# TritonDataCenter/registrar

Hardware: NVIDIA H100
Metric: service-records/sec (higher is better)
Workload: dtype u8

## Files before the change

registrar_b200/csrc/regk_api.cu:

```cuda
#include <cuda_runtime.h>

#include <algorithm>
#include <cstdarg>
#include <cstdio>
#include <cstdlib>
#include <cstring>
#include <map>
#include <mutex>
#include <string>
#include <vector>

#include "../../include/regk.h"
#include "regk_kernels.cuh"
#include "regk_gather.cuh"
#include "regk_peersync.cuh"
#include "regk_service.cuh"
#include "regk_jute.cuh"
#include "regk_decode.cuh"
#include "regk_parents.cuh"
#include "regk_types.hpp"

using namespace regk;

namespace {

thread_local std::string g_create_error;

struct DevBuf {
    void *p = nullptr;
    size_t cap = 0;
};

struct HostBuf {
    void *p = nullptr;
    size_t cap = 0;
};

}

struct regk_ctx {
    int device = 0;
    cudaStream_t own_stream = nullptr;
    cudaStream_t stream = nullptr;
    std::string err;
    int sm_count = 0;
    int max_smem_optin = 0;

    std::vector<std::string> types;
    std::vector<uint8_t> blob_host;
    DevBuf blob_dev;
    uint32_t max_type_q = 0;

    DevBuf in[11];
    DevBuf path_bytes, path_off, json_bytes, json_off, off32_p, off32_j;
    HostBuf h_path_bytes, h_path_off, h_json_bytes, h_json_off, h_running;
    cudaStream_t s_h2d = nullptr, s_d2h = nullptr;
    struct HostSet {
        DevBuf in[11];
        DevBuf path_bytes, path_off, json_bytes, json_off, off32_p, off32_j;
        HostBuf h_path_bytes, h_path_off, h_json_bytes, h_json_off;
        cudaEvent_t e_in = nullptr, e_out = nullptr;
    };
    HostSet hset[2];
    uint64_t hseq = 0;
    uint32_t *h_gather_flag = nullptr;
    double json_mean_seen = 0.0;
    uint64_t json_est_seen = 0;
    bool json_learning = true;
    regk_job job{};
    bool job_bound = false;
    unsigned long long job_seq = 0;
    DevBuf job_bases;
    unsigned long long *h_job_bases = nullptr;
    const uint8_t *last_path_bytes = nullptr;
    const unsigned long long *last_path_off = nullptr;
    uint64_t last_n = 0;
    const uint8_t *last_json_bytes = nullptr;
    const unsigned long long *last_json_off = nullptr;
    uint64_t last_json_n = 0;
// ... 280 lines not shown
            jp.base_out = hp.running + c + 1;
        }
        if (do_path) {
            pp.n = cn;
            pp.rec0 = r0;
            pp.domain_off += r0;
            if (pp.host_off) {
                pp.host_off += r0;
                pp.off_bias = alias ? r0 : 2 * r0;
            } else if (!alias) {
                pp.host_bytes += r0 * (size_t)stride;
                pp.host_limit -= r0 * (uint64_t)stride;
                pp.off_bias = r0 * (uint64_t)(stride + 2);
            } else {
                pp.off_bias = r0;
            }
            pp.out_off += r0;
            pp.tile_total += t0;
            pp.super_total += c * hp.nsuper_chunk;
            const JsonParams side = do_json ? jp : JsonParams{};
            if (alias)
                regk_path_kernel<true, false><<<(unsigned)ct, TILE, path_smem, s>>>(pp, side);
            else
                regk_path_kernel<false, false><<<(unsigned)ct, TILE, path_smem, s>>>(pp, side);
            CK(cudaGetLastError());
            launches++;
        }
        if (do_json) {
            if (!do_path) {
                regk_json_len_kernel<<<(unsigned)std::min<uint64_t>(ct, (uint64_t)ctx->sm_count * 8), TILE, 0, s>>>(jp, (uint32_t)ct);
                CK(cudaGetLastError());
                launches++;
            }
            regk_json_kernel<<<(unsigned)ct, TILE, json_smem, s>>>(jp);
            CK(cudaGetLastError());
            launches++;
            CK(cudaMemcpyAsync(h_running + c + 1, hp.running + c + 1, 8, cudaMemcpyDeviceToHost, s));
        }
        if (c + 1 == hp.nchunks)
            CK(cudaMemcpyAsync(h_status, d_status, sizeof(DevStatus), cudaMemcpyDeviceToHost, s));
        CK(cudaEventRecord(e_done, s));
    }
    h_running[0] = 0;
    for (uint64_t c = 0; c < hp.nchunks; c++) {
        const uint64_t r0 = c * hp.chunk, r1 = std::min(n, r0 + hp.chunk);
        cudaError_t e = cudaEventSynchronize(ctx->pipe_events[3 * c + 1]);
        if (e != cudaSuccess)
            return fail(ctx, REGK_ERR_CUDA, "kernel execution failed: %s", cudaGetErrorString(e));
        const bool last = c + 1 == hp.nchunks;
        if (do_path) {
            const uint64_t lo = path_cf(r0), hi = std::min<uint64_t>(path_cf(r1), hp.path_cap);
            if (hi > lo)
                CK(cudaMemcpyAsync((uint8_t *)ctx->h_path_bytes.p + lo, (uint8_t *)ctx->path_bytes.p + lo, hi - lo,
                    cudaMemcpyDeviceToHost, ctx->s_d2h));
            CK(cudaMemcpyAsync((uint64_t *)ctx->h_path_off.p + r0, (uint64_t *)ctx->path_off.p + r0, (r1 - r0 + (last ? 1 : 0)) * 8,
                cudaMemcpyDeviceToHost, ctx->s_d2h));
        }
        if (do_json) {
            const uint64_t lo = h_running[c], hi = std::min<uint64_t>(h_running[c + 1], hp.json_cap);
            if (hi > lo)
                CK(cudaMemcpyAsync((uint8_t *)ctx->h_json_bytes.p + lo, (uint8_t *)ctx->json_bytes.p + lo, hi - lo,
                    cudaMemcpyDeviceToHost, ctx->s_d2h));
            CK(cudaMemcpyAsync((uint64_t *)ctx->h_json_off.p + r0, (uint64_t *)ctx->json_off.p + r0, (r1 - r0 + (last ? 1 : 0)) * 8,
                cudaMemcpyDeviceToHost, ctx->s_d2h));
        }
    }
    cudaError_t e = cudaStreamSynchronize(ctx->s_d2h);
// ... 226 lines not shown
        cudaStreamDestroy(ctx->own_stream);
    delete ctx;
}

int regk_set_stream(regk_ctx *ctx, void *cuda_stream)
{
    if (!ctx)
        return REGK_ERR_INVALID_ARG;
    if (ctx->pending)
        return fail(ctx, REGK_ERR_STATE, "regk_set_stream: a batch is still pending; call regk_finish first");
    ctx->stream = cuda_stream ? (cudaStream_t)cuda_stream : ctx->own_stream;
    return REGK_OK;
}

int regk_set_option(regk_ctx *ctx, const char *name, int64_t value)
{
    if (!ctx || !name)
        return REGK_ERR_INVALID_ARG;
    static const char *known[] = {"async", "force_generic", "dom_cap", "json_out_cap", "chunk_records", "time_every", "offsets32", nullptr};
    for (const char **k = known; *k; k++)
        if (!strcmp(*k, name)) {
            ctx->opt[name] = value;
            return REGK_OK;
        }
    return fail(ctx, REGK_ERR_INVALID_ARG, "regk_set_option: unknown option '%s'", name);
}

int64_t regk_get_option(const regk_ctx *ctx, const char *name)
{
    if (!ctx || !name)
        return -1;
    if (!strcmp(name, "sm_count"))
        return ctx->sm_count;
    return opt_get(ctx, name, 0);
}

int regk_set_types(regk_ctx *ctx, const char *const *types, const uint32_t *lens, uint32_t ntypes)
{
    if (!ctx || (!types && ntypes))
        return fail(ctx, REGK_ERR_INVALID_ARG, "regk_set_types: NULL argument");
    if (ntypes > 255)
        return fail(ctx, REGK_ERR_INVALID_ARG, "regk_set_types: at most 255 types (type_id is one byte)");
    if (ctx->pending)
        return fail(ctx, REGK_ERR_STATE, "regk_set_types: a batch is still pending");
    CK(cudaSetDevice(ctx->device));
    std::vector<std::string> raw(ntypes);
    for (uint32_t i = 0; i < ntypes; i++)
        raw[i].assign(types[i], lens ? lens[i] : strlen(types[i]));
    std::vector<uint8_t> blob;
    uint32_t maxq = 0;
    std::string why;
    const int brc = build_type_blob(raw, &blob, &maxq, &why);
    if (brc)
        return fail(ctx, brc == 1 ? REGK_ERR_OUT_OF_DOMAIN : REGK_ERR_INVALID_ARG, "regk_set_types: %s", why.c_str());
    int rc = ensure_dev(ctx, ctx->blob_dev, blob.size());
    if (rc)
        return rc;
    CK(cudaMemcpyAsync(ctx->blob_dev.p, blob.data(), blob.size(), cudaMemcpyHostToDevice, ctx->stream));
    CK(cudaStreamSynchronize(ctx->stream));
    ctx->types = raw;
    ctx->blob_host = blob;
    ctx->max_type_q = maxq;
    ctx->json_mean_seen = 0.0;
    ctx->json_learning = true;
    return REGK_OK;
}
// ... 420 lines not shown
        pp.tile_total = (uint32_t *)(wk + totals_p_off);
        pp.super_total = (unsigned long long *)(wk + super_p_off);
        pp.status = d_status;
        pp.dom_limit = dom_len;
        pp.host_limit = host_len;
        pp.force_generic = force_generic;
        const uint64_t mean_dom_tile = std::min<uint64_t>(dom_len, dom_len * TILE / std::max<uint64_t>(n, 1)) + 1;
        uint32_t dom_cap = (uint32_t)opt_get(ctx, "dom_cap", 0);
        if (!dom_cap)
            dom_cap = (uint32_t)std::min<uint64_t>(std::max<uint64_t>(align16(mean_dom_tile * 5 / 4 + 384), 2048), 49152);
        dom_cap = (uint32_t)((dom_cap + 127) & ~127u);
        uint32_t host_cap = 0;
        if (!alias) {
            const uint64_t mean_host_tile = pp.host_off ? std::min<uint64_t>(host_len, host_len * TILE / std::max<uint64_t>(n, 1)) + 1
                                                        : (uint64_t)TILE * b->host_stride;
            host_cap = (uint32_t)std::min<uint64_t>(align16((pp.host_off ? mean_host_tile * 3 / 2 + 512 : mean_host_tile) + 16), 49152);
        }
        const uint32_t out_cap = (uint32_t)align16((uint64_t)dom_cap + host_cap + 2 * TILE + 32);
        path_smem = 16 + (size_t)dom_cap + 32 + dom_cap / 8 + 16 + (alias ? 0 : host_cap + 32) + out_cap + 32;
        if (path_smem > (size_t)ctx->max_smem_optin)
            return fail(ctx, REGK_ERR_INVALID_ARG, "path kernel needs %zu B of shared memory (> %d)", path_smem, ctx->max_smem_optin);
        pp.dom_cap = dom_cap;
        pp.host_cap = host_cap;
        pp.out_cap = out_cap;
        if (smem_attr_needs_raise(ctx->device, alias ? 0 : 1, path_smem)) {
            if (alias) {
                CK(cudaFuncSetAttribute(regk_path_kernel<true, false>, cudaFuncAttributeMaxDynamicSharedMemorySize, (int)path_smem));
                CK(cudaFuncSetAttribute(regk_path_kernel<true, true>, cudaFuncAttributeMaxDynamicSharedMemorySize, (int)path_smem));
            } else {
                CK(cudaFuncSetAttribute(regk_path_kernel<false, false>, cudaFuncAttributeMaxDynamicSharedMemorySize, (int)path_smem));
                CK(cudaFuncSetAttribute(regk_path_kernel<false, true>, cudaFuncAttributeMaxDynamicSharedMemorySize, (int)path_smem));
            }
        }
    }
    JsonParams jp{};
    size_t json_smem = 0;
    if (n && do_json) {
        jp.n = n;
        jp.type_id = (const uint8_t *)dev[4];
        jp.addr_bytes = (const uint8_t *)dev[5];
        jp.addr_off = (const uint32_t *)dev[6];
        jp.ttl = (const int32_t *)dev[7];
        jp.ports_off = (const uint32_t *)dev[8];
        jp.ports = (const uint32_t *)dev[9];
        jp.ports_present = (const uint8_t *)dev[10];
        jp.frag_blob = (const uint8_t *)ctx->blob_dev.p;
        jp.ntypes = (uint32_t)ctx->types.size();
        jp.blob_bytes = (uint32_t)ctx->blob_host.size();
        jp.out_bytes = out_json_bytes;
        jp.out_off = out_json_off;
        jp.out_capacity = out_json_cap;
        if (job) {
            jp.base_in = d_bases + 4;
            fill_peers(jp.peer, J, J.json_bytes, J.json_off);
        }
        jp.tile_total = (uint32_t *)(wk + totals_j_off);
        jp.super_total = (unsigned long long *)(wk + super_j_off);
        jp.status = d_status;
        jp.addr_limit = addr_len;
        jp.ports_limit = ports_len;
        jp.force_generic = force_generic;
        uint32_t out_cap = (uint32_t)opt_get(ctx, "json_out_cap", 0);
        if (!out_cap) {
            uint64_t mean = 42 + 2ull * ctx->max_type_q + (n ? 2 * addr_len / n : 0) + 11 +
                (ports_len ? 11 + (n ? 6 * ports_len / n : 0) : 0) + 2;
            uint64_t tile_bytes = mean * TILE * 9 / 8 + 512;
            slot.json_est = mean;
            slot.json_learned = false;
            if (ctx->json_mean_seen > 0.0 && n >= 4096 && ctx->json_est_seen == mean) {
                const uint64_t seen = (uint64_t)(ctx->json_mean_seen + 1.0);
                if (seen < mean) {
                    tile_bytes = seen * TILE * 17 / 16 + 1024;
                    slot.json_learned = true;
                }
            }
            out_cap = (uint32_t)std::min<uint64_t>(align16(tile_bytes), 98304);
        }
        out_cap = (uint32_t)align16(out_cap);
        jp.out_cap = out_cap;
        json_smem = (size_t)jp.blob_bytes + out_cap + 32;
        if (json_smem > (size_t)ctx->max_smem_optin)
            return fail(ctx, REGK_ERR_INVALID_ARG, "json kernel needs %zu B of shared memory (> %d)", json_smem, ctx->max_smem_optin);
        if (smem_attr_needs_raise(ctx->device, 2, json_smem)) {
            CK(cudaFuncSetAttribute(regk_json_kernel, cudaFuncAttributeMaxDynamicSharedMemorySize, (int)json_smem));
        }
    }

    if (pipelined) {
        HostPipe hp;
        hp.chunk = chunk_records;
        hp.nchunks = nchunks;
        hp.nsuper_chunk = nsuper_chunk;
        hp.running = (unsigned long long *)(wk + running_off);
        hp.path_cap = path_cap;
        hp.json_cap = json_cap;
        for (int i = 0; i < 11; i++) {
            hp.src[i] = src[i];
            hp.dev[i] = need[i] && src[i] ? ctx->in[i].p : nullptr;
        }
        rc = run_pipelined(ctx, b, res, pp, path_smem, jp, json_smem, hp);
        if (rc == REGK_OK) {
            ctx->last_path_bytes = do_path ? pp.out_bytes : nullptr;
            ctx->last_path_off = do_path ? pp.out_off : nullptr;
            ctx->last_n = do_path ? n : 0;
            ctx->last_json_bytes = do_json ? jp.out_bytes : nullptr;
            ctx->last_json_off = do_json ? jp.out_off : nullptr;
            ctx->last_json_n = do_json ? n : 0;
            ctx->last_host_off = pp.host_off;
            ctx->last_host_stride = pp.host_stride;
            ctx->last_alias = alias;
        }
        if (rc != REGK_ERR_STATE + 100)
            return rc;
        for (int i = 0; i < 11; i++)
            if (dev[i] && sz[i])
                CK(cudaMemcpyAsync(ctx->in[i].p, src[i], sz[i], cudaMemcpyHostToDevice, s));
        CK(cudaMemsetAsync(wk, 0, work_bytes, s));
// ... 20 lines not shown
        launches++;
    }
    if (timed)
        CK(cudaEventRecord(slot.ev[0], s));
    if (n && do_path) {
        if (alias)
            regk_path_kernel<true, false><<<(unsigned)ntiles, TILE, path_smem, s>>>(pp, fused_len ? jp : JsonParams{});
        else
            regk_path_kernel<false, false><<<(unsigned)ntiles, TILE, path_smem, s>>>(pp, fused_len ? jp : JsonParams{});
        CK(cudaGetLastError());
        launches++;
        slot.path_params = pp;
        slot.path_smem = path_smem;
        slot.path_alias = alias;
        slot.did_path = true;
    }
    if (timed)
        CK(cudaEventRecord(slot.ev[1], s));
    if (job) {
        if ((rc = launch_exchange(ctx, 0, 0, n ? jp.super_total : nullptr, n ? (uint32_t)nsuper_chunk : 0, d_bases + 4,
                 (unsigned long long *)J.json_off[J.rank] + J.n_total)))
            return rc;
        launches++;
    }
    if (n && do_json) {
        if (!fused_len) {
            const unsigned len_grid = (unsigned)std::min<uint64_t>(ntiles, (uint64_t)ctx->sm_count * 8);
            regk_json_len_kernel<<<len_grid, TILE, 0, s>>>(jp, (uint32_t)ntiles);
            CK(cudaGetLastError());
            launches++;
        }
        if (timed)
            CK(cudaEventRecord(slot.ev[2], s));
        regk_json_kernel<<<(unsigned)ntiles, TILE, json_smem, s>>>(jp);
        CK(cudaGetLastError());
        launches++;
    } else if (timed) {
        CK(cudaEventRecord(slot.ev[2], s));
    }
    slot.off32 = !out_dev && !job && n && opt_get(ctx, "offsets32", 0) != 0;
    if (slot.off32) {
        if (do_path && (rc = narrow_offsets(ctx, o_path_off.p, hs ? hs->off32_p : ctx->off32_p, n, s)))
            return rc;
        if (do_json && (rc = narrow_offsets(ctx, o_json_off.p, hs ? hs->off32_j : ctx->off32_j, n, s)))
            return rc;
    }
    CK(cudaEventRecord(slot.ev[3], s));
    if (job) {
        if ((rc = launch_exchange(ctx, 0, 0, nullptr, 0, nullptr, nullptr)))
            return rc;
        launches++;
        CK(cudaEventRecord(slot.ev[5], s));
    }
    if (ring >= 0) {
        CK(cudaStreamWaitEvent(ctx->s_side, job ? slot.ev[5] : slot.ev[3], 0));
        CK(cudaMemcpyAsync(slot.h_status, d_status, sizeof(DevStatus), cudaMemcpyDeviceToHost, ctx->s_side));
        if (job)
            CK(cudaMemcpyAsync(ctx->h_job_bases + 8 * (ctx->seq % regk_ctx::NSLOTS), d_bases, 64, cudaMemcpyDeviceToHost, ctx->s_side));
        CK(cudaEventRecord(slot.ev[4], ctx->s_side));
        CK(cudaMemsetAsync(wk, 0, work_bytes, ctx->s_side));
        CK(cudaEventRecord(ctx->ws_clean[ring], ctx->s_side));
        ctx->ws_clean_bytes[ring] = work_bytes;
        slot.ring = ring;
    } else {
        CK(cudaMemcpyAsync(slot.h_status, d_status, sizeof(DevStatus), cudaMemcpyDeviceToHost, s));
        CK(cudaEventRecord(slot.ev[4], s));
        slot.ring = -1;
// ... 687 lines not shown
```

registrar_b200/csrc/regk_kernels.cuh:

```cuda
#ifndef REGK_KERNELS_CUH
#define REGK_KERNELS_CUH

#include <cuda_runtime.h>
#include <stdint.h>

#include "../../include/regk.h"
#include "regk_core.cuh"

namespace regk {

#ifndef REGK_TILE
#define REGK_TILE 128
#endif
#ifndef REGK_MINB_PATH
#define REGK_MINB_PATH 12
#endif
#ifndef REGK_MINB_JSON
#define REGK_MINB_JSON 12
#endif
constexpr int TILE = REGK_TILE;
constexpr int WARPS = TILE / 32;

struct DevStatus {
    uint32_t bad_bits;
    uint32_t overflow;
    unsigned long long first_bad;
    unsigned long long path_total;
    unsigned long long json_total;
    uint32_t needs_exact;
    uint32_t generic_tiles;
};

__device__ __forceinline__ uint4 ldg_nc_v4(const void *p)
{
    uint4 r;
    asm volatile("ld.global.nc.L1::no_allocate.v4.u32 {%0,%1,%2,%3}, [%4];"
                 : "=r"(r.x), "=r"(r.y), "=r"(r.z), "=r"(r.w) : "l"(p));
    return r;
}

__device__ __forceinline__ void stg_v4(void *p, const uint4 &v)
{
    asm volatile("st.global.L1::no_allocate.v4.u32 [%0], {%1,%2,%3,%4};"
                 ::"l"(p), "r"(v.x), "r"(v.y), "r"(v.z), "r"(v.w) : "memory");
}

__device__ __forceinline__ uint32_t smem_u32(const void *p)
{
    return (uint32_t)__cvta_generic_to_shared(p);
}

// ... 15 lines not shown
}

__device__ __forceinline__ void mbar_wait(uint64_t *bar, uint32_t parity)
{
    uint32_t done;
    do {
        asm volatile("{\n\t.reg .pred p;\n\tmbarrier.try_wait.parity.shared::cta.b64 p, [%1], %2;\n\tselp.u32 %0, 1, 0, p;\n\t}"
                     : "=r"(done) : "r"(smem_u32(bar)), "r"(parity) : "memory");
    } while (!done);
}

__device__ __forceinline__ void stage_in(uint8_t *smem, const uint8_t *src, uint64_t g0, uint64_t g1,
    uint64_t limit)
{
    const uint64_t a0 = g0 & ~15ull;
    const uint8_t *base = src + a0;
    const uint32_t nchunks = (uint32_t)((g1 - a0 + 15) >> 4);
    const uint32_t safe = limit > a0 ? (uint32_t)min((uint64_t)nchunks, (limit - a0) >> 4) : 0u;
    for (uint32_t c = threadIdx.x; c < nchunks; c += TILE) {
        if (c < safe) {
            reinterpret_cast<uint4 *>(smem)[c] = ldg_nc_v4(base + 16u * c);
        } else {
            for (uint32_t k = 0; k < 16; k++)
                smem[16u * c + k] = (a0 + 16ull * c + k < limit) ? base[16u * c + k] : (uint8_t)0;
        }
    }
}

__device__ __forceinline__ void fence_proxy_async()
{
    asm volatile("fence.proxy.async.shared::cta;" ::: "memory");
}

__device__ __forceinline__ void flush_out(uint8_t *gout, const uint8_t *smem, uint64_t gbase, uint32_t total)
{
    const uint64_t a0 = gbase & ~15ull;
    const uint32_t lo = (uint32_t)(gbase - a0);
    const uint32_t hi = lo + total;
    uint32_t body_lo = (lo + 15u) & ~15u, body_hi = hi & ~15u;
    if (body_hi <= body_lo)
        body_lo = body_hi = hi;
    const uint32_t t = threadIdx.x;
    if (t == 0 && body_hi > body_lo) {
        const uint32_t src = (uint32_t)__cvta_generic_to_shared(smem + body_lo);
        asm volatile("cp.async.bulk.global.shared::cta.bulk_group [%0], [%1], %2;"
                     ::"l"(gout + a0 + body_lo), "r"(src), "r"(body_hi - body_lo) : "memory");
        asm volatile("cp.async.bulk.commit_group;" ::: "memory");
    }
    if (t < 32) {
        const uint32_t i = lo + t;
        if (i < body_lo)
            gout[a0 + i] = smem[i];
    } else if (t < 48) {
        const uint32_t i = body_hi + (t - 32);
        if (i < hi)
            gout[a0 + i] = smem[i];
    }
    if (t == 0 && body_hi > body_lo)
        asm volatile("cp.async.bulk.wait_group.read 0;" ::: "memory");
}

struct PeerDst {
    uint32_t n;
    uint32_t job;
    uint8_t *bytes[REGK_MAX_PEERS - 1];
    unsigned long long *off[REGK_MAX_PEERS - 1];
};

__device__ __forceinline__ void peer_tables(const PeerDst &pd, uint8_t **s_pb, unsigned long long **s_po)
{
    const uint32_t t = threadIdx.x;
    if (t < REGK_MAX_PEERS - 1) {
        uint8_t *b = nullptr;
        unsigned long long *o = nullptr;
        #pragma unroll
        for (int q = 0; q < REGK_MAX_PEERS - 1; q++)
            if (t == (uint32_t)q) {
                b = pd.bytes[q];
                o = pd.off[q];
            }
        s_pb[t] = b;
        s_po[t] = o;
    }
}

__device__ __forceinline__ void store_block_part(uint8_t *gblk, const uint8_t *sblk, uint32_t lo, uint32_t hi)
{
    while (lo < hi) {
        const uint32_t left = hi - lo;
        if (!(lo & 7u) && left >= 8u) {
            *reinterpret_cast<uint64_t *>(gblk + lo) = *reinterpret_cast<const uint64_t *>(sblk + lo);
            lo += 8u;
        } else if (!(lo & 3u) && left >= 4u) {
            *reinterpret_cast<uint32_t *>(gblk + lo) = *reinterpret_cast<const uint32_t *>(sblk + lo);
            lo += 4u;
        } else if (!(lo & 1u) && left >= 2u) {
            *reinterpret_cast<uint16_t *>(gblk + lo) = *reinterpret_cast<const uint16_t *>(sblk + lo);
            lo += 2u;
        } else {
            gblk[lo] = sblk[lo];
            lo += 1u;
        }
    }
}

__device__ __forceinline__ void bulk_s2g(uint8_t *gdst, const uint8_t *smem_src, uint32_t bytes)
{
    asm volatile("cp.async.bulk.global.shared::cta.bulk_group [%0], [%1], %2;"
                 ::"l"(gdst), "r"(smem_u32(smem_src)), "r"(bytes) : "memory");
}

__device__ __forceinline__ void flush_out_job(uint8_t *gout, uint8_t *const *s_pb, uint32_t npeers, const uint8_t *smem,
    uint64_t gbase, uint32_t total)
{
    if (threadIdx.x != 0 || total == 0)
        return;
    const uint64_t a0 = gbase & ~15ull;
    const uint32_t lo = (uint32_t)(gbase - a0);
    const uint32_t hi = lo + total;
    const uint32_t b_first = lo >> 4, b_last = (hi - 1u) >> 4;
    for (uint32_t d = 0; d <= npeers; d++) {
        uint8_t *g = (d == 0 ? gout : s_pb[d - 1]) + a0;
        if (b_first == b_last) {
            store_block_part(g + 16u * b_first, smem + 16u * b_first, lo & 15u, ((hi - 1u) & 15u) + 1u);
        } else {
            uint32_t body_lo = lo, body_hi = hi;
            if (lo & 15u) {
                store_block_part(g + 16u * b_first, smem + 16u * b_first, lo & 15u, 16u);
                body_lo = 16u * (b_first + 1u);
            }
            if (hi & 15u) {
                store_block_part(g + 16u * b_last, smem + 16u * b_last, 0u, hi & 15u);
                body_hi = 16u * b_last;
            }
            if (body_hi > body_lo)
                bulk_s2g(g + body_lo, smem + body_lo, body_hi - body_lo);
        }
    }
    asm volatile("cp.async.bulk.commit_group;" ::: "memory");
    asm volatile("cp.async.bulk.wait_group.read 0;" ::: "memory");
}

__device__ __forceinline__ void copy_range_to_peers(const uint8_t *gown, uint8_t *const *s_pb, uint32_t npeers, uint64_t gbase,
    uint32_t total)
{
    const uint64_t end = gbase + total;
    uint64_t body_lo = (gbase + 15ull) & ~15ull, body_hi = end & ~15ull;
    if (body_hi <= body_lo)
        body_lo = body_hi = end;
    for (uint64_t b = body_lo + 16ull * threadIdx.x; b < body_hi; b += 16ull * TILE) {
        const uint4 v = *reinterpret_cast<const uint4 *>(gown + b);
        for (uint32_t q = 0; q < npeers; q++)
            stg_v4(s_pb[q] + b, v);
    }
    for (uint64_t i = gbase + threadIdx.x; i < body_lo; i += TILE)
        for (uint32_t q = 0; q < npeers; q++)
            s_pb[q][i] = gown[i];
    for (uint64_t i = body_hi + threadIdx.x; i < end; i += TILE)
        for (uint32_t q = 0; q < npeers; q++)
            s_pb[q][i] = gown[i];
}

template <typename T>
__device__ __forceinline__ T block_scan(T *warp_sum , T v, T *total)
{
    const uint32_t lane = threadIdx.x & 31u, warp = threadIdx.x >> 5;
    T incl = v;
    #pragma unroll
    for (int d = 1; d < 32; d <<= 1) {
        T up = __shfl_up_sync(0xFFFFFFFFu, incl, d);
        if (lane >= (uint32_t)d)
            incl += up;
    }
// ... 42 lines not shown

__device__ __forceinline__ void report_bad(DevStatus *st, uint32_t bad, uint64_t rec)
{
    if (bad) {
        atomicOr(&st->bad_bits, bad);
        atomicMax(&st->first_bad, ~(unsigned long long)rec);
    }
}


struct JsonParams {
    uint64_t n;
    const uint8_t *type_id;
    const uint8_t *addr_bytes;
    const uint32_t *addr_off;
    const int32_t *ttl;
    const uint32_t *ports_off;
    const uint32_t *ports;
    const uint8_t *ports_present;
    const uint8_t *frag_blob;
    uint32_t ntypes;
    uint32_t blob_bytes;
    uint8_t *out_bytes;
    unsigned long long *out_off;
    uint64_t out_capacity;
    uint64_t rec0;
    const unsigned long long *base_in;
    unsigned long long *base_out;
    uint32_t *tile_total;
    unsigned long long *super_total;
    DevStatus *status;
    uint64_t addr_limit, ports_limit;
    uint32_t out_cap;
    uint32_t force_generic;
    PeerDst peer;
};

struct JsonMeta {
    uint32_t tid, a0, al, p0, k;
    int32_t ttl;
    bool has_ttl, has_ports;
    uint32_t bad;
};

__device__ __forceinline__ JsonMeta json_meta(const JsonParams &p, uint64_t r)
{
    JsonMeta m;
    m.bad = 0;
    m.tid = p.type_id[r];
    if (m.tid >= p.ntypes) {
        m.bad |= BAD_TYPE_ID;
        m.tid = 0;
    }
    m.a0 = p.addr_off[r];
    uint32_t a1 = p.addr_off[r + 1];
    if (a1 < m.a0 || a1 > p.addr_limit) {
        m.bad |= BAD_TOO_LARGE;
        a1 = m.a0 = 0;
    }
    m.al = a1 - m.a0;
    if (m.al == 0)
        m.bad |= BAD_ADDR_BYTE;
    m.ttl = p.ttl ? p.ttl[r] : INT32_MIN;
    m.has_ttl = m.ttl != INT32_MIN;
    m.p0 = 0;
    m.k = 0;
    if (p.ports_off) {
        m.p0 = p.ports_off[r];
        uint32_t p1 = p.ports_off[r + 1];
        if (p1 < m.p0 || p1 > p.ports_limit) {
            m.bad |= BAD_TOO_LARGE;
            p1 = m.p0 = 0;
        }
        m.k = p1 - m.p0;
    }
    m.has_ports = p.ports_present ? (p.ports_present[r] != 0) : (m.k > 0);
    if (!m.has_ports)
        m.k = 0;
    return m;
}

__device__ __forceinline__ uint32_t json_meta_len(const JsonParams &p, const JsonMeta &m, const TypeFrag &tf)
{
    const uint32_t *pp = p.ports + m.p0;
    const uint32_t k = m.k;
    uint32_t port_digits = 0;
    if (k) {
        const uint32_t v0 = pp[0], v1 = k > 1u ? pp[1] : 0u, v2 = k > 2u ? pp[2] : 0u, v3 = k > 3u ? pp[3] : 0u;
        port_digits = ndigits_u32(v0) + (k > 1u ? ndigits_u32(v1) : 0u) + (k > 2u ? ndigits_u32(v2) : 0u) +
                      (k > 3u ? ndigits_u32(v3) : 0u);
        for (uint32_t i = 4; i < k; i++)
            port_digits += ndigits_u32(pp[i]);
    }
    return json_length(tf.f1_len, tf.f2_len, m.al, m.has_ttl, m.ttl, m.has_ports, m.k, port_digits);
}


struct PathParams {
    uint64_t n;
    const uint8_t *domain_bytes;
    const uint32_t *domain_off;
    const uint8_t *host_bytes;
    const uint32_t *host_off;
    uint32_t host_stride;
    uint8_t *out_bytes;
    unsigned long long *out_off;
    uint64_t out_capacity;
    uint64_t rec0;
    uint64_t off_bias;
    uint32_t exact;
    uint32_t *tile_total;
    unsigned long long *super_total;
    DevStatus *status;
    uint64_t dom_limit, host_limit;
    uint32_t dom_cap, host_cap, out_cap;
    uint32_t force_generic;
    const unsigned long long *bias_in;
// ... 12 lines not shown
template <bool ALIAS>
__global__ void __launch_bounds__(TILE) regk_path_len_kernel(const PathParams p)
{
    const uint32_t tile = blockIdx.x, t = threadIdx.x;
    const uint64_t r0 = (uint64_t)tile * TILE;
    const uint32_t nrec = (uint32_t)min((uint64_t)TILE, p.n - r0);
    uint32_t len = 0;
    if (t < nrec) {
        const uint64_t r = r0 + t;
        const uint32_t d0 = p.domain_off[r], d1 = p.domain_off[r + 1];
        const uint32_t L = (d1 >= d0 && d1 <= p.dom_limit) ? d1 - d0 : 0;
        uint32_t H = 0;
        if (!ALIAS) {
            if (p.host_off) {
                const uint32_t a = p.host_off[r], b = p.host_off[r + 1];
                H = b >= a ? b - a : 0;
            } else {
                H = p.host_stride;
            }
        }
        const GuardedWords dsrc{reinterpret_cast<const uint32_t *>(p.domain_bytes)};
        len = path_length(scan_domain(dsrc, d0, L), L, H, ALIAS);
    }
    #pragma unroll
    for (int d = 16; d > 0; d >>= 1)
        len += __shfl_xor_sync(0xFFFFFFFFu, len, d);
    if ((t & 31u) == 0)
        add_tile_total(p.tile_total, p.super_total, tile, len);
}

__device__ __forceinline__ void payload_length_side_job(const JsonParams &jp, const JsonMeta &jm, const TypeFrag &jtf,
    bool live, uint32_t tile)
{
    uint32_t jl = live ? json_meta_len(jp, jm, jtf) : 0;
    #pragma unroll
    for (int d = 16; d > 0; d >>= 1)
        jl += __shfl_xor_sync(0xFFFFFFFFu, jl, d);
    if ((threadIdx.x & 31u) == 0)
        add_tile_total(jp.tile_total, jp.super_total, tile, jl);
}

struct TilePlan {
    unsigned long long tile_base;
    unsigned long long HB0;
    uint32_t D0, D1, HA1;
    uint32_t nd, nh;
    uint32_t host_span;
    uint32_t tile_total;
    uint32_t flags;
};
enum : uint32_t { PLAN_BROKEN = 1, PLAN_FITS = 2, PLAN_BULK = 4, PLAN_ROOM = 8 };

template <bool ALIAS, bool EXACT>
__global__ void __launch_bounds__(TILE, REGK_MINB_PATH) regk_path_kernel(const PathParams p, const JsonParams jp)
{
    extern __shared__ __align__(16) uint8_t smem[];
    __shared__ uint32_t warp_sum[WARPS];
    __shared__ __align__(8) uint64_t s_bar;
    __shared__ TilePlan s_plan;
    __shared__ uint8_t *s_pb[REGK_MAX_PEERS - 1];
    __shared__ unsigned long long *s_po[REGK_MAX_PEERS - 1];
    const uint32_t npeers = p.peer.n;
    if (npeers)
        peer_tables(p.peer, s_pb, s_po);
    uint8_t *s_dom = smem + 16;
    uint8_t *s_bits = s_dom + p.dom_cap + 32;
    uint8_t *s_host = s_bits + p.dom_cap / 8 + 16;
    uint8_t *s_out = s_host + (ALIAS ? 0 : p.host_cap + 32);

    const uint32_t tile = blockIdx.x;
    const uint32_t t = threadIdx.x;
    const uint64_t r0 = (uint64_t)tile * TILE;
    const uint32_t nrec = (uint32_t)min((uint64_t)TILE, p.n - r0);
    const bool live = t < nrec;
    const uint32_t tl = live ? t : 0u;
    const uint64_t r = r0 + tl;
    constexpr bool exact = EXACT;
    const bool var_host = !ALIAS && p.host_off != nullptr;
    const uint32_t per_rec = ALIAS ? 1u : 2u;

    if (t == 0) {
        mbar_init(&s_bar, 1);
        TilePlan q;
        q.D0 = p.domain_off[r0];
// ... 179 lines not shown
            ByteSink sink;
            sink.init(p.out_bytes + tile_base + local);
            emit_path<ALIAS>(dsrc, d0, L, hsrc, hoff, H, sink);
        }
        if (npeers && room) {
            __syncthreads();
            copy_range_to_peers(p.out_bytes, s_pb, npeers, tile_base, tile_total);
        }
    }
    if (!room && !(flags & PLAN_BROKEN) && t == 0)
        atomicOr(&p.status->overflow, 1u);
    if (live)
        report_bad(p.status, bad, p.rec0 + r);
    if (r0 + nrec == p.n && t == 0) {
        if (p.peer.job) {
            p.status->path_total = tile_base + tile_total - (p.bias_in ? *p.bias_in : 0ull) - p.off_bias;
        } else {
            p.out_off[p.n] = tile_base + tile_total;
            p.status->path_total = tile_base + tile_total;
        }
    }
}


__global__ void __launch_bounds__(TILE) regk_json_len_kernel(const JsonParams p, uint32_t ntiles)
{
    const uint32_t t = threadIdx.x, lane = t & 31u;
    for (uint32_t tile = blockIdx.x; tile < ntiles; tile += gridDim.x) {
        const uint64_t r = (uint64_t)tile * TILE + t;
        uint32_t len = 0;
        if (r < p.n) {
            const JsonMeta m = json_meta(p, r);
            const TypeFrag tf = reinterpret_cast<const TypeFrag *>(p.frag_blob)[m.tid];
            len = json_meta_len(p, m, tf);
        }
        #pragma unroll
        for (int d = 16; d > 0; d >>= 1)
            len += __shfl_xor_sync(0xFFFFFFFFu, len, d);
        if (lane == 0)
            add_tile_total(p.tile_total, p.super_total, tile, len);
    }
}

struct JsonPlan {
    unsigned long long tile_base;
    uint32_t tile_total;
    uint32_t flags;
};

__global__ void __launch_bounds__(TILE, REGK_MINB_JSON) regk_json_kernel(const JsonParams p)
{
    extern __shared__ __align__(16) uint8_t smem[];
    __shared__ uint32_t warp_sum[WARPS];
    __shared__ __align__(8) uint64_t s_bar;
    __shared__ JsonPlan s_plan;
    __shared__ uint8_t *s_pb[REGK_MAX_PEERS - 1];
    __shared__ unsigned long long *s_po[REGK_MAX_PEERS - 1];
    const uint32_t npeers = p.peer.n;
    if (npeers)
        peer_tables(p.peer, s_pb, s_po);
    uint8_t *s_blob = smem;
    uint8_t *s_out = smem + p.blob_bytes;

    const uint32_t t = threadIdx.x;
    const uint32_t tile = blockIdx.x;
    const uint64_t r0 = (uint64_t)tile * TILE;
    const uint32_t nrec = (uint32_t)min((uint64_t)TILE, p.n - r0);
    const bool live = t < nrec;
    const uint64_t r = r0 + (live ? t : 0);

    if (t < 32) {
        if (t == 0) {
            mbar_init(&s_bar, 1);
            mbar_expect_tx(&s_bar, p.blob_bytes);
            bulk_g2s(s_blob, p.frag_blob, p.blob_bytes, &s_bar);
        }
        const unsigned long long b = tile_base_from_totals(p.tile_total, p.super_total, tile) + (p.base_in ? *p.base_in : 0ull);
        if (t == 0) {
            JsonPlan q;
            q.tile_base = b;
            q.tile_total = p.tile_total[tile];
            q.flags = (b + q.tile_total <= p.out_capacity ? PLAN_ROOM : 0u) |
                (!p.force_generic && q.tile_total + 16u <= p.out_cap ? PLAN_FITS : 0u);
            s_plan = q;
        }
    }

    const JsonMeta m = json_meta(p, r);
    uint32_t bad = m.bad;
    const uint32_t a0 = m.a0, al = m.al, k = m.k;

    const GuardedWords asrc{reinterpret_cast<const uint32_t *>(p.addr_bytes)};
    uint32_t aw[4] = {0, 0, 0, 0};
    {
        const uint32_t n16 = al < 16u ? al : 16u;
        const uint32_t sh = (a0 & 3u) * 8u;
        uint32_t wi = a0 >> 2;
        uint32_t lo = n16 ? asrc.word(wi) : 0u;
        #pragma unroll
        for (int w = 0; w < 4; w++) {
            if (n16 > 4u * w) {
                const uint32_t nb = min(4u, n16 - 4u * w);
                const uint32_t hi = asrc.word_hi(wi + 1, sh + 8u * nb > 32u || n16 > 4u * (w + 1));
                const uint32_t keep = low_bytes(nb);
                aw[w] = funnel_r(lo, hi, sh) & keep;
                if (addr_word_bad(aw[w], keep))
                    bad |= BAD_ADDR_BYTE;
                lo = hi;
                wi++;
            }
        }
        for (uint32_t i = a0 + 16u; i < a0 + al; i++) {
            const uint32_t c = p.addr_bytes[i];
            if (c < 0x20u || c >= 0x80u || c == 0x22u || c == 0x5Cu)
                bad |= BAD_ADDR_BYTE;
        }
    }
    const TypeFrag tf = reinterpret_cast<const TypeFrag *>(p.frag_blob)[m.tid];
    const uint32_t len = live ? json_meta_len(p, m, tf) : 0;
    uint32_t tot;
    const uint32_t local = block_scan<uint32_t>(warp_sum, len, &tot);
    mbar_wait(&s_bar, 0);
    const unsigned long long tile_base = s_plan.tile_base;
    const uint32_t tile_total = s_plan.tile_total;
    const uint32_t flags = s_plan.flags;
    if (live) {
        p.out_off[r] = tile_base + local;
        for (uint32_t q = 0; q < npeers; q++)
            s_po[q][r] = tile_base + local;
    }

    const PaddedWords blob{reinterpret_cast<const uint32_t *>(s_blob)};
    const uint32_t *ports = p.ports + m.p0;
    auto port = [ports](uint32_t i) { return ports[i]; };
    if (!(flags & PLAN_ROOM)) {
        if (t == 0)
            atomicOr(&p.status->overflow, 1u);
    } else if (flags & PLAN_FITS) {
        WordSink sink;
        sink.init(reinterpret_cast<uint32_t *>(s_out), local + ((uint32_t)tile_base & 15u));
        if (live)
            emit_json(blob, tf, aw, asrc, a0, al, m.has_ttl, m.ttl, m.has_ports, k, port, sink);
        __syncthreads();
        if (live)
            sink.tail();
        fence_proxy_async();
        __syncthreads();
        if (npeers)
            flush_out_job(p.out_bytes, s_pb, npeers, s_out, tile_base, tile_total);
        else
            flush_out(p.out_bytes, s_out, tile_base, tile_total);
    } else {
        if (t == 0)
            atomicAdd(&p.status->generic_tiles, 1u);
        if (live) {
            ByteSink sink;
            sink.init(p.out_bytes + tile_base + local);
            emit_json(blob, tf, aw, asrc, a0, al, m.has_ttl, m.ttl, m.has_ports, k, port, sink);
        }
        if (npeers) {
            __syncthreads();
            copy_range_to_peers(p.out_bytes, s_pb, npeers, tile_base, tile_total);
        }
    }
    if (live)
        report_bad(p.status, bad, p.rec0 + r);
    if (r0 + nrec == p.n && t == 0) {
        if (p.peer.job) {
            p.status->json_total = tile_base + tile_total - (p.base_in ? *p.base_in : 0ull);
        } else {
            p.out_off[p.n] = tile_base + tile_total;
            p.status->json_total = tile_base + tile_total;
            if (p.base_out)
                *p.base_out = tile_base + tile_total;
        }
    }
}

}
#endif
```

Baseline: 6.346 billion.

## Make JSON kernel persistent with double-buffered bulk-copy staging of tile inputs

After: 6.687 billion (median of 6 runs). +5.4%, better.

```diff
diff --git a/registrar_b200/csrc/regk_api.cu b/registrar_b200/csrc/regk_api.cu
--- a/registrar_b200/csrc/regk_api.cu
+++ b/registrar_b200/csrc/regk_api.cu
@@ -45,6 +45,8 @@
     std::string err;
     int sm_count = 0;
     int max_smem_optin = 0;
+    int path_ctas = 0, json_ctas = 0;
+    size_t path_ctas_smem = 0, json_ctas_smem = 0;
 
     std::vector<std::string> types;
     std::vector<uint8_t> blob_host;
@@ -391,7 +393,7 @@
                 CK(cudaGetLastError());
                 launches++;
             }
-            regk_json_kernel<<<(unsigned)ct, TILE, json_smem, s>>>(jp);
+            regk_json_kernel<<<(unsigned)std::min<uint64_t>(ct, (uint64_t)ctx->sm_count * ctx->json_ctas), TILE, json_smem, s>>>(jp);
             CK(cudaGetLastError());
             launches++;
             CK(cudaMemcpyAsync(h_running + c + 1, hp.running + c + 1, 8, cudaMemcpyDeviceToHost, s));
@@ -684,6 +686,10 @@
         return -1;
     if (!strcmp(name, "sm_count"))
         return ctx->sm_count;
+    if (!strcmp(name, "path_ctas_per_sm"))
+        return ctx->path_ctas;
+    if (!strcmp(name, "json_ctas_per_sm"))
+        return ctx->json_ctas;
     return opt_get(ctx, name, 0);
 }
 
@@ -1170,6 +1176,13 @@
                 CK(cudaFuncSetAttribute(regk_path_kernel<false, true>, cudaFuncAttributeMaxDynamicSharedMemorySize, (int)path_smem));
             }
         }
+        if (path_smem != ctx->path_ctas_smem || !ctx->path_ctas) {
+            if (alias)
+                CK(cudaOccupancyMaxActiveBlocksPerMultiprocessor(&ctx->path_ctas, regk_path_kernel<true, false>, TILE, path_smem));
+            else
+                CK(cudaOccupancyMaxActiveBlocksPerMultiprocessor(&ctx->path_ctas, regk_path_kernel<false, false>, TILE, path_smem));
+            ctx->path_ctas_smem = path_smem;
+        }
     }
     JsonParams jp{};
     size_t json_smem = 0;
@@ -1216,11 +1229,20 @@
         }
         out_cap = (uint32_t)align16(out_cap);
         jp.out_cap = out_cap;
-        json_smem = (size_t)jp.blob_bytes + out_cap + 32;
+        const uint64_t tile_addr = addr_len * TILE / n, tile_ports = 4 * ports_len * TILE / n;
+        jp.addr_cap = (uint32_t)std::min<uint64_t>(align16(tile_addr * 17 / 16 + 64), 16384);
+        jp.ports_cap = jp.ports_off ? (uint32_t)std::min<uint64_t>(align16(tile_ports * 3 / 2 + 128), 16384) : 0u;
+        json_smem = (size_t)jp.blob_bytes + out_cap + 32 + 2 * (size_t)json_stage_bytes(jp.addr_cap, jp.ports_cap);
         if (json_smem > (size_t)ctx->max_smem_optin)
             return fail(ctx, REGK_ERR_INVALID_ARG, "json kernel needs %zu B of shared memory (> %d)", json_smem, ctx->max_smem_optin);
         if (smem_attr_needs_raise(ctx->device, 2, json_smem)) {
             CK(cudaFuncSetAttribute(regk_json_kernel, cudaFuncAttributeMaxDynamicSharedMemorySize, (int)json_smem));
+        }
+        if (json_smem != ctx->json_ctas_smem || !ctx->json_ctas) {
+            CK(cudaOccupancyMaxActiveBlocksPerMultiprocessor(&ctx->json_ctas, regk_json_kernel, TILE, json_smem));
+            if (!ctx->json_ctas)
+                return fail(ctx, REGK_ERR_INVALID_ARG, "json kernel: no CTA fits an SM with %zu B of shared memory", json_smem);
+            ctx->json_ctas_smem = json_smem;
         }
     }
 
@@ -1307,7 +1329,7 @@
         }
         if (timed)
             CK(cudaEventRecord(slot.ev[2], s));
-        regk_json_kernel<<<(unsigned)ntiles, TILE, json_smem, s>>>(jp);
+        regk_json_kernel<<<(unsigned)std::min<uint64_t>(ntiles, (uint64_t)ctx->sm_count * ctx->json_ctas), TILE, json_smem, s>>>(jp);
         CK(cudaGetLastError());
         launches++;
     } else if (timed) {
diff --git a/registrar_b200/csrc/regk_kernels.cuh b/registrar_b200/csrc/regk_kernels.cuh
--- a/registrar_b200/csrc/regk_kernels.cuh
+++ b/registrar_b200/csrc/regk_kernels.cuh
@@ -13,10 +13,10 @@
 #define REGK_TILE 128
 #endif
 #ifndef REGK_MINB_PATH
-#define REGK_MINB_PATH 12
+#define REGK_MINB_PATH 8
 #endif
 #ifndef REGK_MINB_JSON
-#define REGK_MINB_JSON 12
+#define REGK_MINB_JSON 8
 #endif
 constexpr int TILE = REGK_TILE;
 constexpr int WARPS = TILE / 32;
@@ -98,7 +98,7 @@
     asm volatile("fence.proxy.async.shared::cta;" ::: "memory");
 }
 
-__device__ __forceinline__ void flush_out(uint8_t *gout, const uint8_t *smem, uint64_t gbase, uint32_t total)
+__device__ __forceinline__ void flush_out(uint8_t *gout, const uint8_t *smem, uint64_t gbase, uint32_t total, bool wait = true)
 {
     const uint64_t a0 = gbase & ~15ull;
     const uint32_t lo = (uint32_t)(gbase - a0);
@@ -122,7 +122,7 @@
         if (i < hi)
             gout[a0 + i] = smem[i];
     }
-    if (t == 0 && body_hi > body_lo)
+    if (wait && t == 0 && body_hi > body_lo)
         asm volatile("cp.async.bulk.wait_group.read 0;" ::: "memory");
 }
 
@@ -177,7 +177,7 @@
 }
 
 __device__ __forceinline__ void flush_out_job(uint8_t *gout, uint8_t *const *s_pb, uint32_t npeers, const uint8_t *smem,
-    uint64_t gbase, uint32_t total)
+    uint64_t gbase, uint32_t total, bool wait = true)
 {
     if (threadIdx.x != 0 || total == 0)
         return;
@@ -204,7 +204,8 @@
         }
     }
     asm volatile("cp.async.bulk.commit_group;" ::: "memory");
-    asm volatile("cp.async.bulk.wait_group.read 0;" ::: "memory");
+    if (wait)
+        asm volatile("cp.async.bulk.wait_group.read 0;" ::: "memory");
 }
 
 __device__ __forceinline__ void copy_range_to_peers(const uint8_t *gown, uint8_t *const *s_pb, uint32_t npeers, uint64_t gbase,
@@ -313,6 +314,7 @@
     DevStatus *status;
     uint64_t addr_limit, ports_limit;
     uint32_t out_cap;
+    uint32_t addr_cap, ports_cap;
     uint32_t force_generic;
     PeerDst peer;
 };
@@ -324,17 +326,24 @@
     uint32_t bad;
 };
 
-__device__ __forceinline__ JsonMeta json_meta(const JsonParams &p, uint64_t r)
+struct MetaPtrs {
+    const uint8_t *type_id;
+    const uint32_t *addr_off;
+    const uint32_t *ports_off;
+};
+
+__device__ __forceinline__ JsonMeta json_meta_at(const JsonParams &p, const MetaPtrs &e, uint64_t i, uint64_t r,
+    int32_t ttl)
 {
     JsonMeta m;
     m.bad = 0;
-    m.tid = p.type_id[r];
+    m.tid = e.type_id[i];
     if (m.tid >= p.ntypes) {
         m.bad |= BAD_TYPE_ID;
         m.tid = 0;
     }
-    m.a0 = p.addr_off[r];
-    uint32_t a1 = p.addr_off[r + 1];
+    m.a0 = e.addr_off[i];
+    uint32_t a1 = e.addr_off[i + 1];
     if (a1 < m.a0 || a1 > p.addr_limit) {
         m.bad |= BAD_TOO_LARGE;
         a1 = m.a0 = 0;
@@ -342,13 +351,13 @@
     m.al = a1 - m.a0;
     if (m.al == 0)
         m.bad |= BAD_ADDR_BYTE;
-    m.ttl = p.ttl ? p.ttl[r] : INT32_MIN;
+    m.ttl = ttl;
     m.has_ttl = m.ttl != INT32_MIN;
     m.p0 = 0;
     m.k = 0;
-    if (p.ports_off) {
-        m.p0 = p.ports_off[r];
-        uint32_t p1 = p.ports_off[r + 1];
+    if (e.ports_off) {
+        m.p0 = e.ports_off[i];
+        uint32_t p1 = e.ports_off[i + 1];
         if (p1 < m.p0 || p1 > p.ports_limit) {
             m.bad |= BAD_TOO_LARGE;
             p1 = m.p0 = 0;
@@ -361,9 +370,13 @@
     return m;
 }
 
-__device__ __forceinline__ uint32_t json_meta_len(const JsonParams &p, const JsonMeta &m, const TypeFrag &tf)
-{
-    const uint32_t *pp = p.ports + m.p0;
+__device__ __forceinline__ JsonMeta json_meta(const JsonParams &p, uint64_t r)
+{
+    return json_meta_at(p, MetaPtrs{p.type_id, p.addr_off, p.ports_off}, r, r, p.ttl ? p.ttl[r] : INT32_MIN);
+}
+
+__device__ __forceinline__ uint32_t json_meta_len(const uint32_t *pp, const JsonMeta &m, const TypeFrag &tf)
+{
     const uint32_t k = m.k;
     uint32_t port_digits = 0;
     if (k) {
@@ -442,7 +455,7 @@
 __device__ __forceinline__ void payload_length_side_job(const JsonParams &jp, const JsonMeta &jm, const TypeFrag &jtf,
     bool live, uint32_t tile)
 {
-    uint32_t jl = live ? json_meta_len(jp, jm, jtf) : 0;
+    uint32_t jl = live ? json_meta_len(jp.ports + jm.p0, jm, jtf) : 0;
     #pragma unroll
     for (int d = 16; d > 0; d >>= 1)
         jl += __shfl_xor_sync(0xFFFFFFFFu, jl, d);
@@ -459,7 +472,7 @@
     uint32_t tile_total;
     uint32_t flags;
 };
-enum : uint32_t { PLAN_BROKEN = 1, PLAN_FITS = 2, PLAN_BULK = 4, PLAN_ROOM = 8 };
+enum : uint32_t { PLAN_BROKEN = 1, PLAN_FITS = 2, PLAN_BULK = 4, PLAN_ROOM = 8, PLAN_STAGED = 16, PLAN_OVER = 32 };
 
 template <bool ALIAS, bool EXACT>
 __global__ void __launch_bounds__(TILE, REGK_MINB_PATH) regk_path_kernel(const PathParams p, const JsonParams jp)
@@ -705,7 +718,7 @@
         if (r < p.n) {
             const JsonMeta m = json_meta(p, r);
             const TypeFrag tf = reinterpret_cast<const TypeFrag *>(p.frag_blob)[m.tid];
-            len = json_meta_len(p, m, tf);
+            len = json_meta_len(p.ports + m.p0, m, tf);
         }
         #pragma unroll
         for (int d = 16; d > 0; d >>= 1)
@@ -715,18 +728,81 @@
     }
 }
 
+constexpr uint32_t JST_TYPE = 0, JST_AOFF = TILE, JST_POFF = JST_AOFF + 4 * (TILE + 4), JST_PORTS = JST_POFF + 4 * (TILE + 4);
+
+__device__ __forceinline__ int32_t tile_ttl(const JsonParams &p, uint32_t tile)
+{
+    const uint64_t r0 = (uint64_t)tile * TILE;
+    return p.ttl ? p.ttl[r0 + (r0 + threadIdx.x < p.n ? threadIdx.x : 0u)] : INT32_MIN;
+}
+
+__host__ __device__ constexpr uint32_t json_stage_bytes(uint32_t addr_cap, uint32_t ports_cap)
+{
+    return addr_cap ? JST_PORTS + ports_cap + addr_cap : 0u;
+}
+
 struct JsonPlan {
     unsigned long long tile_base;
     uint32_t tile_total;
     uint32_t flags;
+    uint32_t A0, A1, P0, P1;
 };
+
+__device__ __forceinline__ void json_plan_tile(const JsonParams &p, uint32_t tile, uint8_t *stage, uint64_t *bar, JsonPlan *dst)
+{
+    const uint32_t t = threadIdx.x;
+    const uint64_t r0 = (uint64_t)tile * TILE;
+    JsonPlan q;
+    q.A0 = q.A1 = q.P0 = q.P1 = 0;
+    const bool aligned = (((uintptr_t)p.type_id | (uintptr_t)p.addr_off | (uintptr_t)p.ports_off |
+                           (uintptr_t)p.ports | (uintptr_t)p.addr_bytes) & 15u) == 0;
+    const bool candidate = p.addr_cap && !p.force_generic && aligned && r0 + TILE + 3 <= p.n;
+    if (t == 0 && candidate) {
+        q.A0 = p.addr_off[r0];
+        q.A1 = p.addr_off[r0 + TILE];
+        if (p.ports_off) {
+            q.P0 = p.ports_off[r0];
+            q.P1 = p.ports_off[r0 + TILE];
+        }
+    }
+    const unsigned long long b = tile_base_from_totals(p.tile_total, p.super_total, tile) + (p.base_in ? *p.base_in : 0ull);
+    if (t != 0)
+        return;
+    const uint64_t a_lo = q.A0 & ~15u, a_hi = (q.A1 + 15ull) & ~15ull;
+    const uint64_t p_lo = (4ull * q.P0) & ~15ull, p_hi = (4ull * q.P1 + 15ull) & ~15ull;
+    const bool ok = candidate && q.A1 >= q.A0 && a_hi <= p.addr_limit &&
+        (!p.ports_off || (q.P1 >= q.P0 && p_hi <= 4ull * p.ports_limit));
+    const bool fit = ok && a_hi - a_lo <= p.addr_cap && p_hi - p_lo <= p.ports_cap;
+    uint32_t bytes = 0;
+    if (fit)
+        bytes = TILE + 4u * (TILE + 4) + (p.ports_off ? 4u * (TILE + 4) : 0u) +
+            (uint32_t)(a_hi - a_lo) + (uint32_t)(p_hi - p_lo);
+    fence_proxy_async();
+    mbar_expect_tx(bar, bytes);
+    if (fit) {
+        bulk_g2s(stage + JST_TYPE, p.type_id + r0, TILE, bar);
+        bulk_g2s(stage + JST_AOFF, p.addr_off + r0, 4u * (TILE + 4), bar);
+        if (p.ports_off)
+            bulk_g2s(stage + JST_POFF, p.ports_off + r0, 4u * (TILE + 4), bar);
+        if (p_hi > p_lo)
+            bulk_g2s(stage + JST_PORTS, reinterpret_cast<const uint8_t *>(p.ports) + p_lo, (uint32_t)(p_hi - p_lo), bar);
+        if (a_hi > a_lo)
+            bulk_g2s(stage + JST_PORTS + p.ports_cap, p.addr_bytes + a_lo, (uint32_t)(a_hi - a_lo), bar);
+    }
+    q.tile_base = b;
+    q.tile_total = p.tile_total[tile];
+    q.flags = (b + q.tile_total <= p.out_capacity ? PLAN_ROOM : 0u) |
+        (!p.force_generic && q.tile_total + 16u <= p.out_cap ? PLAN_FITS : 0u) |
+        (fit ? PLAN_STAGED : 0u) | (ok && !fit ? PLAN_OVER : 0u);
+    *dst = q;
+}
 
 __global__ void __launch_bounds__(TILE, REGK_MINB_JSON) regk_json_kernel(const JsonParams p)
 {
     extern __shared__ __align__(16) uint8_t smem[];
     __shared__ uint32_t warp_sum[WARPS];
-    __shared__ __align__(8) uint64_t s_bar;
-    __shared__ JsonPlan s_plan;
+    __shared__ __align__(8) uint64_t s_bar[3];
+    __shared__ JsonPlan s_plan[2];
     __shared__ uint8_t *s_pb[REGK_MAX_PEERS - 1];
     __shared__ unsigned long long *s_po[REGK_MAX_PEERS - 1];
     const uint32_t npeers = p.peer.n;
@@ -734,120 +810,147 @@
         peer_tables(p.peer, s_pb, s_po);
     uint8_t *s_blob = smem;
     uint8_t *s_out = smem + p.blob_bytes;
+    uint8_t *s_stage = s_out + p.out_cap + 32;
+    const uint32_t stage_bytes = json_stage_bytes(p.addr_cap, p.ports_cap);
 
     const uint32_t t = threadIdx.x;
-    const uint32_t tile = blockIdx.x;
-    const uint64_t r0 = (uint64_t)tile * TILE;
-    const uint32_t nrec = (uint32_t)min((uint64_t)TILE, p.n - r0);
-    const bool live = t < nrec;
-    const uint64_t r = r0 + (live ? t : 0);
-
-    if (t < 32) {
-        if (t == 0) {
-            mbar_init(&s_bar, 1);
-            mbar_expect_tx(&s_bar, p.blob_bytes);
-            bulk_g2s(s_blob, p.frag_blob, p.blob_bytes, &s_bar);
-        }
-        const unsigned long long b = tile_base_from_totals(p.tile_total, p.super_total, tile) + (p.base_in ? *p.base_in : 0ull);
-        if (t == 0) {
-            JsonPlan q;
-            q.tile_base = b;
-            q.tile_total = p.tile_total[tile];
-            q.flags = (b + q.tile_total <= p.out_capacity ? PLAN_ROOM : 0u) |
-                (!p.force_generic && q.tile_total + 16u <= p.out_cap ? PLAN_FITS : 0u);
-            s_plan = q;
-        }
-    }
-
-    const JsonMeta m = json_meta(p, r);
-    uint32_t bad = m.bad;
-    const uint32_t a0 = m.a0, al = m.al, k = m.k;
-
-    const GuardedWords asrc{reinterpret_cast<const uint32_t *>(p.addr_bytes)};
-    uint32_t aw[4] = {0, 0, 0, 0};
-    {
-        const uint32_t n16 = al < 16u ? al : 16u;
-        const uint32_t sh = (a0 & 3u) * 8u;
-        uint32_t wi = a0 >> 2;
-        uint32_t lo = n16 ? asrc.word(wi) : 0u;
-        #pragma unroll
-        for (int w = 0; w < 4; w++) {
-            if (n16 > 4u * w) {
-                const uint32_t nb = min(4u, n16 - 4u * w);
-                const uint32_t hi = asrc.word_hi(wi + 1, sh + 8u * nb > 32u || n16 > 4u * (w + 1));
-                const uint32_t keep = low_bytes(nb);
-                aw[w] = funnel_r(lo, hi, sh) & keep;
-                if (addr_word_bad(aw[w], keep))
+    const uint32_t ntiles = (uint32_t)((p.n + TILE - 1) / TILE);
+    if (t == 0) {
+        mbar_init(&s_bar[0], 1);
+        mbar_init(&s_bar[1], 1);
+        mbar_init(&s_bar[2], 1);
+        mbar_expect_tx(&s_bar[2], p.blob_bytes);
+        bulk_g2s(s_blob, p.frag_blob, p.blob_bytes, &s_bar[2]);
+    }
+    if (t < 32)
+        json_plan_tile(p, blockIdx.x, s_stage, &s_bar[0], &s_plan[0]);
+    __syncthreads();
+    mbar_wait(&s_bar[2], 0);
+    const PaddedWords blob{reinterpret_cast<const uint32_t *>(s_blob)};
+    const TypeFrag *s_frag = reinterpret_cast<const TypeFrag *>(s_blob);
+    int32_t ttl_next = tile_ttl(p, blockIdx.x);
+
+    for (uint32_t j = 0, tile = blockIdx.x; tile < ntiles; j++, tile += gridDim.x) {
+        const uint32_t s = j & 1u;
+        const uint8_t *stage = s_stage + s * stage_bytes;
+        if (t < 32 && tile + gridDim.x < ntiles)
+            json_plan_tile(p, tile + gridDim.x, s_stage + (s ^ 1u) * stage_bytes, &s_bar[s ^ 1u], &s_plan[s ^ 1u]);
+        const uint32_t flags = s_plan[s].flags;
+        const uint32_t A0 = s_plan[s].A0, A1 = s_plan[s].A1, P0 = s_plan[s].P0, P1 = s_plan[s].P1;
+        const uint64_t r0 = (uint64_t)tile * TILE;
+        const uint32_t nrec = (uint32_t)min((uint64_t)TILE, p.n - r0);
+        const bool live = t < nrec;
+        const uint32_t tl = live ? t : 0u;
+        const uint64_t r = r0 + tl;
+        const bool staged = flags & PLAN_STAGED;
+        const int32_t ttl = ttl_next;
+        if (tile + gridDim.x < ntiles)
+            ttl_next = tile_ttl(p, tile + gridDim.x);
+        mbar_wait(&s_bar[s], (j >> 1) & 1u);
+
+        const JsonMeta m = staged ?
+            json_meta_at(p, MetaPtrs{stage + JST_TYPE, reinterpret_cast<const uint32_t *>(stage + JST_AOFF),
+                                     p.ports_off ? reinterpret_cast<const uint32_t *>(stage + JST_POFF) : nullptr}, tl, r, ttl) :
+            json_meta_at(p, MetaPtrs{p.type_id, p.addr_off, p.ports_off}, r, r, ttl);
+        uint32_t bad = m.bad;
+        const uint32_t a0 = m.a0, al = m.al, k = m.k;
+        const uint8_t *abytes = p.addr_bytes;
+        const uint32_t *pvals = p.ports;
+        if (staged) {
+            if (a0 >= A0 && a0 + al <= A1)
+                abytes = stage + JST_PORTS + p.ports_cap - (A0 & ~15u);
+            if (m.p0 >= P0 && m.p0 + k <= P1)
+                pvals = reinterpret_cast<const uint32_t *>(stage + JST_PORTS) - (P0 & ~3u);
+        }
+
+        const GuardedWords asrc{reinterpret_cast<const uint32_t *>(abytes)};
+        uint32_t aw[4] = {0, 0, 0, 0};
+        {
+            const uint32_t n16 = al < 16u ? al : 16u;
+            const uint32_t sh = (a0 & 3u) * 8u;
+            uint32_t wi = a0 >> 2;
+            uint32_t lo = n16 ? asrc.word(wi) : 0u;
+            #pragma unroll
+            for (int w = 0; w < 4; w++) {
+                if (n16 > 4u * w) {
+                    const uint32_t nb = min(4u, n16 - 4u * w);
+                    const uint32_t hi = asrc.word_hi(wi + 1, sh + 8u * nb > 32u || n16 > 4u * (w + 1));
+                    const uint32_t keep = low_bytes(nb);
+                    aw[w] = funnel_r(lo, hi, sh) & keep;
+                    if (addr_word_bad(aw[w], keep))
+                        bad |= BAD_ADDR_BYTE;
+                    lo = hi;
+                    wi++;
+                }
+            }
+            for (uint32_t i = a0 + 16u; i < a0 + al; i++) {
+                const uint32_t c = abytes[i];
+                if (c < 0x20u || c >= 0x80u || c == 0x22u || c == 0x5Cu)
                     bad |= BAD_ADDR_BYTE;
-                lo = hi;
-                wi++;
             }
         }
-        for (uint32_t i = a0 + 16u; i < a0 + al; i++) {
-            const uint32_t c = p.addr_bytes[i];
-            if (c < 0x20u || c >= 0x80u || c == 0x22u || c == 0x5Cu)
-                bad |= BAD_ADDR_BYTE;
-        }
-    }
-    const TypeFrag tf = reinterpret_cast<const TypeFrag *>(p.frag_blob)[m.tid];
-    const uint32_t len = live ? json_meta_len(p, m, tf) : 0;
-    uint32_t tot;
-    const uint32_t local = block_scan<uint32_t>(warp_sum, len, &tot);
-    mbar_wait(&s_bar, 0);
-    const unsigned long long tile_base = s_plan.tile_base;
-    const uint32_t tile_total = s_plan.tile_total;
-    const uint32_t flags = s_plan.flags;
-    if (live) {
-        p.out_off[r] = tile_base + local;
-        for (uint32_t q = 0; q < npeers; q++)
-            s_po[q][r] = tile_base + local;
-    }
-
-    const PaddedWords blob{reinterpret_cast<const uint32_t *>(s_blob)};
-    const uint32_t *ports = p.ports + m.p0;
-    auto port = [ports](uint32_t i) { return ports[i]; };
-    if (!(flags & PLAN_ROOM)) {
+        const TypeFrag tf = s_frag[m.tid];
+        const uint32_t len = live ? json_meta_len(pvals + m.p0, m, tf) : 0;
         if (t == 0)
-            atomicOr(&p.status->overflow, 1u);
-    } else if (flags & PLAN_FITS) {
-        WordSink sink;
-        sink.init(reinterpret_cast<uint32_t *>(s_out), local + ((uint32_t)tile_base & 15u));
+            asm volatile("cp.async.bulk.wait_group.read 0;" ::: "memory");
+        uint32_t tot;
+        const uint32_t local = block_scan<uint32_t>(warp_sum, len, &tot);
+        const unsigned long long tile_base = s_plan[s].tile_base;
+        const uint32_t tile_total = s_plan[s].tile_total;
+        if (live) {
+            p.out_off[r] = tile_base + local;
+            for (uint32_t q = 0; q < npeers; q++)
+                s_po[q][r] = tile_base + local;
+        }
+
+        const uint32_t *ports = pvals + m.p0;
+        auto port = [ports](uint32_t i) { return ports[i]; };
+        if (!(flags & PLAN_ROOM)) {
+            if (t == 0)
+                atomicOr(&p.status->overflow, 1u);
+        } else if (flags & PLAN_FITS) {
+            WordSink sink;
+            sink.init(reinterpret_cast<uint32_t *>(s_out), local + ((uint32_t)tile_base & 15u));
+            if (live)
+                emit_json(blob, tf, aw, asrc, a0, al, m.has_ttl, m.ttl, m.has_ports, k, port, sink);
+            __syncthreads();
+            if (live)
+                sink.tail();
+            fence_proxy_async();
+            __syncthreads();
+            if (npeers)
+                flush_out_job(p.out_bytes, s_pb, npeers, s_out, tile_base, tile_total, false);
+            else
+                flush_out(p.out_bytes, s_out, tile_base, tile_total, false);
+        } else {
+            if (live) {
+                ByteSink sink;
+                sink.init(p.out_bytes + tile_base + local);
+                emit_json(blob, tf, aw, asrc, a0, al, m.has_ttl, m.ttl, m.has_ports, k, port, sink);
+            }
+            if (npeers) {
+                __syncthreads();
+                copy_range_to_peers(p.out_bytes, s_pb, npeers, tile_base, tile_total);
+            }
+        }
+        if (t == 0 && ((flags & PLAN_OVER) || ((flags & PLAN_ROOM) && !(flags & PLAN_FITS))))
+            atomicAdd(&p.status->generic_tiles, 1u);
         if (live)
-            emit_json(blob, tf, aw, asrc, a0, al, m.has_ttl, m.ttl, m.has_ports, k, port, sink);
+            report_bad(p.status, bad, p.rec0 + r);
+        if (r0 + nrec == p.n && t == 0) {
+            if (p.peer.job) {
+                p.status->json_total = tile_base + tile_total - (p.base_in ? *p.base_in : 0ull);
+            } else {
+                p.out_off[p.n] = tile_base + tile_total;
+                p.status->json_total = tile_base + tile_total;
+                if (p.base_out)
+                    *p.base_out = tile_base + tile_total;
+            }
+        }
         __syncthreads();
-        if (live)
-            sink.tail();
-        fence_proxy_async();
-        __syncthreads();
-        if (npeers)
-            flush_out_job(p.out_bytes, s_pb, npeers, s_out, tile_base, tile_total);
-        else
-            flush_out(p.out_bytes, s_out, tile_base, tile_total);
-    } else {
-        if (t == 0)
-            atomicAdd(&p.status->generic_tiles, 1u);
-        if (live) {
-            ByteSink sink;
-            sink.init(p.out_bytes + tile_base + local);
-            emit_json(blob, tf, aw, asrc, a0, al, m.has_ttl, m.ttl, m.has_ports, k, port, sink);
-        }
-        if (npeers) {
-            __syncthreads();
-            copy_range_to_peers(p.out_bytes, s_pb, npeers, tile_base, tile_total);
-        }
-    }
-    if (live)
-        report_bad(p.status, bad, p.rec0 + r);
-    if (r0 + nrec == p.n && t == 0) {
-        if (p.peer.job) {
-            p.status->json_total = tile_base + tile_total - (p.base_in ? *p.base_in : 0ull);
-        } else {
-            p.out_off[p.n] = tile_base + tile_total;
-            p.status->json_total = tile_base + tile_total;
-            if (p.base_out)
-                *p.base_out = tile_base + tile_total;
-        }
-    }
+    }
+    if (t == 0)
+        asm volatile("cp.async.bulk.wait_group.read 0;" ::: "memory");
 }
 
 }
```
